# BillyXYB/TransEditor

Hardware: AMD Instinct MI355X
Metric: 256x256 images/sec/GPU, G+D fwd+bwd, batch 16; 1/2/4/8-GPU scaling (higher is better)
Workload: dtype f32

## Files before the change

transeditor_amd/csrc/rgb.hip:

```cpp
#include "te_common.h"

namespace {

constexpr int KMAX = 512;
constexpr int NOUT = 3;

__global__ __launch_bounds__(256) void rgb_fwd_kernel(float* __restrict__ out, const float* __restrict__ x,
                                                      const float* __restrict__ w, const float* __restrict__ isc,
                                                      const float* __restrict__ bias, float wscale, int K, int HW) {
    __shared__ float ws[NOUT][KMAX];
    const int b = blockIdx.y, tid = threadIdx.x;
    for (int k = tid; k < K; k += 256) {
        const float s = (isc ? isc[(size_t)b * K + k] : 1.f) * wscale;
#pragma unroll
        for (int o = 0; o < NOUT; ++o) ws[o][k] = w[o * K + k] * s;
    }
    __syncthreads();
    const int HW4 = HW >> 2;
    const int p4 = blockIdx.x * 256 + tid;
    if (p4 >= HW4) return;
    const float4* xp = reinterpret_cast<const float4*>(x + (size_t)b * K * HW) + p4;
    float4 acc[NOUT];
#pragma unroll
    for (int o = 0; o < NOUT; ++o) acc[o] = make_float4(0.f, 0.f, 0.f, 0.f);
#pragma unroll 8
    for (int k = 0; k < K; ++k) {
        const float4 v = xp[(size_t)k * HW4];
#pragma unroll
        for (int o = 0; o < NOUT; ++o) {
            const float c = ws[o][k];
            acc[o].x += c * v.x; acc[o].y += c * v.y; acc[o].z += c * v.z; acc[o].w += c * v.w;
        }
    }
#pragma unroll
    for (int o = 0; o < NOUT; ++o) {
        const float bb = bias ? bias[o] : 0.f;
        acc[o].x += bb; acc[o].y += bb; acc[o].z += bb; acc[o].w += bb;
        reinterpret_cast<float4*>(out + ((size_t)b * NOUT + o) * HW)[p4] = acc[o];
    }
}

__global__ __launch_bounds__(256) void rgb_dgrad_kernel(float* __restrict__ gx, const float* __restrict__ g,
                                                        const float* __restrict__ w, const float* __restrict__ isc,
                                                        float wscale, int K, int HW, const float* __restrict__ bias = nullptr,
                                                        int act = 0) {
    __shared__ float ws[NOUT][KMAX];
    const int b = blockIdx.y, tid = threadIdx.x;
    for (int k = tid; k < K; k += 256) {
        const float s = (isc ? isc[(size_t)b * K + k] : 1.f) * wscale;
#pragma unroll
        for (int o = 0; o < NOUT; ++o) ws[o][k] = w[o * K + k] * s;
    }
    __syncthreads();
    const int HW4 = HW >> 2;
    const int p4 = blockIdx.x * 256 + tid;
    if (p4 >= HW4) return;
    float4 gv[NOUT];
#pragma unroll
    for (int o = 0; o < NOUT; ++o) gv[o] = reinterpret_cast<const float4*>(g + ((size_t)b * NOUT + o) * HW)[p4];
    float4* op = reinterpret_cast<float4*>(gx + (size_t)b * K * HW) + p4;
    const float gain = act == 3 ? 1.4142135623730951f : 1.f;
#pragma unroll 4
    for (int k = 0; k < K; ++k) {
        const float c0 = ws[0][k], c1 = ws[1][k], c2 = ws[2][k];
        const float bb = bias ? bias[k] : 0.f;
        float4 r;
        r.x = c0 * gv[0].x + c1 * gv[1].x + c2 * gv[2].x + bb;
        r.y = c0 * gv[0].y + c1 * gv[1].y + c2 * gv[2].y + bb;
        r.z = c0 * gv[0].z + c1 * gv[1].z + c2 * gv[2].z + bb;
        r.w = c0 * gv[0].w + c1 * gv[1].w + c2 * gv[2].w + bb;
        if (act >= 3) {
            r.x = (r.x > 0.f ? r.x : 0.2f * r.x) * gain; r.y = (r.y > 0.f ? r.y : 0.2f * r.y) * gain;
            r.z = (r.z > 0.f ? r.z : 0.2f * r.z) * gain; r.w = (r.w > 0.f ? r.w : 0.2f * r.w) * gain;
        }
        op[(size_t)k * HW4] = r;
    }
}

inline int rgb_pow2(int v) { int p = 1; while (p < v) p <<= 1; return p; }
inline int rgb_tile_px(int K) { return std::max(32, std::min(256, 8192 / rgb_pow2(K))); }

template <bool SUM>
__global__ __launch_bounds__(256) void rgb_wgrad_kernel(float* __restrict__ slabs, const float* __restrict__ g,
                                                        const float* __restrict__ x, int K, int HW, int S, int TPX, int lgTPX, int K2) {
    constexpr int NROW = SUM ? NOUT + 1 : NOUT;
    extern __shared__ __attribute__((aligned(16))) float smem[];
    float* xl = smem;
    float* gl = smem + K * (TPX + 1);
    const int b = blockIdx.y, c = blockIdx.x, tid = threadIdx.x;
    const int ntile = (HW + TPX - 1) / TPX;
    const int t0 = (int)((int64_t)ntile * c / S), t1 = (int)((int64_t)ntile * (c + 1) / S);
    const float* xb = x + (size_t)b * K * HW;
    const float* gb = g + (size_t)b * NOUT * HW;
    const bool vec4 = (HW & 3) == 0 && ((reinterpret_cast<uintptr_t>(x) & 15) == 0);
    const int parts = K2 >= 256 ? 1 : 256 / K2;
    const int kk = K2 >= 256 ? tid : (tid & (K2 - 1)), part = K2 >= 256 ? 0 : tid / K2;
    const int nh = K2 > 256 ? 2 : 1;
    float acc[2][NOUT + 1] = {{0.f, 0.f, 0.f, 0.f}, {0.f, 0.f, 0.f, 0.f}};
    for (int tl = t0; tl < t1; ++tl) {
        const int p0 = tl * TPX;
        __syncthreads();
        if (vec4) {
            for (int e0 = 0; e0 < K * TPX; e0 += 256 * 8 * 4) {
                float4 st[8];
#pragma unroll
                for (int j = 0; j < 8; ++j) {
                    const int e = e0 + 4 * (tid + 256 * j), k = e >> lgTPX, pp = e & (TPX - 1);
                    const bool ok = e < K * TPX && p0 + pp < HW;
                    st[j] = ok ? *reinterpret_cast<const float4*>(xb + (size_t)k * HW + p0 + pp) : make_float4(0.f, 0.f, 0.f, 0.f);
                }
#pragma unroll
                for (int j = 0; j < 8; ++j) {
                    const int e = e0 + 4 * (tid + 256 * j), k = e >> lgTPX, pp = e & (TPX - 1);
                    if (e < K * TPX) {
                        float* d = xl + k * (TPX + 1) + pp;
                        d[0] = st[j].x; d[1] = st[j].y; d[2] = st[j].z; d[3] = st[j].w;
                    }
                }
            }
        } else {
            for (int e0 = 0; e0 < K * TPX; e0 += 256 * 8) {
                float st[8];
#pragma unroll
                for (int j = 0; j < 8; ++j) {
                    const int e = e0 + tid + 256 * j, k = e >> lgTPX, pp = e & (TPX - 1);
                    const bool ok = e < K * TPX && p0 + pp < HW;
                    const float v = xb[ok ? (size_t)k * HW + p0 + pp : 0];
                    st[j] = ok ? v : 0.f;
                }
#pragma unroll
                for (int j = 0; j < 8; ++j) {
                    const int e = e0 + tid + 256 * j, k = e >> lgTPX, pp = e & (TPX - 1);
                    if (e < K * TPX) xl[k * (TPX + 1) + pp] = st[j];
                }
            }
        }
        for (int e = tid; e < NOUT * TPX; e += 256) {
            const int o = e >> lgTPX, pp = e & (TPX - 1);
            gl[e] = (p0 + pp < HW) ? gb[(size_t)o * HW + p0 + pp] : 0.f;
        }
        __syncthreads();
        for (int h = 0; h < nh; ++h) {
            const int k = kk + 256 * h;
            if (k < K) {
#pragma unroll 4
                for (int pp = part; pp < TPX; pp += parts) {
                    const float xv = xl[k * (TPX + 1) + pp];
#pragma unroll
                    for (int o = 0; o < NOUT; ++o) acc[h][o] += gl[o * TPX + pp] * xv;
                    if (SUM) acc[h][NOUT] += xv;
                }
            }
        }
    }
    float* sl = slabs + ((size_t)b * S + c) * NROW * K;
    if (parts > 1) {
        __syncthreads();
        float* red = smem;
#pragma unroll
        for (int o = 0; o < NROW; ++o) red[(part * NROW + o) * K2 + kk] = acc[0][o];
        __syncthreads();
        if (part == 0 && kk < K) {
#pragma unroll
            for (int o = 0; o < NROW; ++o) {
                float a = 0.f;
                for (int q = 0; q < parts; ++q) a += red[(q * NROW + o) * K2 + kk];
                sl[o * K + kk] = a;
            }
        }
        return;
    }
    for (int h = 0; h < nh; ++h) {
        const int k = kk + 256 * h;
        if (k < K) {
#pragma unroll
            for (int o = 0; o < NROW; ++o) sl[o * K + k] = acc[h][o];
        }
    }
}

inline bool ok_shape(int K, int HW) { return K > 0 && K <= KMAX && HW > 0 && (HW & 3) == 0; }

}

extern "C" int te_rgb_supported(int M, int K, int HW) { return (M == NOUT && ok_shape(K, HW)) ? 1 : 0; }

extern "C" int te_rgb_fwd_f32(float* out, const float* x, const float* w, const float* isc, const float* bias, float wscale,
                              int B, int K, int HW, te_stream_t stream_) {
    TE_REQUIRE(out && x && w, TE_ERR_NULL, "te_rgb_fwd_f32: NULL pointer");
    TE_REQUIRE(B > 0 && ok_shape(K, HW), TE_ERR_UNSUPPORTED, "te_rgb_fwd_f32: need K <= 512 and H*W %% 4 == 0");
    dim3 grid((unsigned)te::cdiv(HW / 4, 256), (unsigned)B);
    rgb_fwd_kernel<<<grid, 256, 0, (hipStream_t)stream_>>>(out, x, w, isc, bias, wscale, K, HW);
    return te::launch_status("te_rgb_fwd_f32");
}

extern "C" int te_rgb_dgrad_f32(float* gx, const float* g, const float* w, const float* isc, float wscale, int B, int K,
                                int HW, te_stream_t stream_) {
    TE_REQUIRE(gx && g && w, TE_ERR_NULL, "te_rgb_dgrad_f32: NULL pointer");
    TE_REQUIRE(B > 0 && ok_shape(K, HW), TE_ERR_UNSUPPORTED, "te_rgb_dgrad_f32: need K <= 512 and H*W %% 4 == 0");
    dim3 grid((unsigned)te::cdiv(HW / 4, 256), (unsigned)B);
    rgb_dgrad_kernel<<<grid, 256, 0, (hipStream_t)stream_>>>(gx, g, w, isc, wscale, K, HW);
    return te::launch_status("te_rgb_dgrad_f32");
}

extern "C" int te_rgb_expand_f32(float* out, const float* x3, const float* w, const float* bias, int act, float wscale, int B,
                                 int K, int HW, te_stream_t stream_) {
    TE_REQUIRE(out && x3 && w, TE_ERR_NULL, "te_rgb_expand_f32: NULL pointer");
    TE_REQUIRE(B > 0 && ok_shape(K, HW), TE_ERR_UNSUPPORTED, "te_rgb_expand_f32: need K <= 512 and H*W %% 4 == 0");
    TE_REQUIRE(act == 0 || act == 3 || act == 4, TE_ERR_UNSUPPORTED, "te_rgb_expand_f32: act must be 0, 3 or 4");
    dim3 grid((unsigned)te::cdiv(HW / 4, 256), (unsigned)B);
    rgb_dgrad_kernel<<<grid, 256, 0, (hipStream_t)stream_>>>(out, x3, w, nullptr, wscale, K, HW, bias, act);
    return te::launch_status("te_rgb_expand_f32");
}

extern "C" int te_rgb_wgrad_slab_count(int B, int K, int HW) {
    if (B <= 0 || K <= 0 || HW <= 0) return TE_ERR_SHAPE;
    const int64_t ntile = te::cdiv(HW, rgb_tile_px(K));
    int64_t S = te::cdiv(4 * te::kNumCU, B);
    return (int)std::max<int64_t>(1, std::min<int64_t>(S, ntile));
}

extern "C" int te_rgb_wgrad_f32(float* slabs, const float* g, const float* x, int B, int K, int HW, int S, te_stream_t stream_) {
    TE_REQUIRE(slabs && g && x, TE_ERR_NULL, "te_rgb_wgrad_f32: NULL pointer");
    TE_REQUIRE(B > 0 && K > 0 && K <= KMAX && HW > 0 && S > 0, TE_ERR_UNSUPPORTED, "te_rgb_wgrad_f32: need 0 < K <= 512");
    const int TPX = rgb_tile_px(K), K2 = rgb_pow2(K);
    int lg = 0;
    while ((1 << lg) < TPX) ++lg;
    const size_t lds = sizeof(float) * std::max<size_t>((size_t)K * (TPX + 1) + NOUT * TPX, (size_t)256 * (NOUT + 1));
    static std::atomic<uint64_t> attr_done{0};
    te::allow_big_lds(attr_done, (const void*)rgb_wgrad_kernel<false>, 96 * 1024);
    dim3 grid((unsigned)S, (unsigned)B);
    rgb_wgrad_kernel<false><<<grid, 256, lds, (hipStream_t)stream_>>>(slabs, g, x, K, HW, S, TPX, lg, K2);
    return te::launch_status("te_rgb_wgrad_f32");
}

extern "C" int te_rgb_wgrad_sum_f32(float* slabs, const float* g, const float* x, int B, int K, int HW, int S, te_stream_t stream_) {
    TE_REQUIRE(slabs && g && x, TE_ERR_NULL, "te_rgb_wgrad_sum_f32: NULL pointer");
    TE_REQUIRE(B > 0 && K > 0 && K <= KMAX && HW > 0 && S > 0, TE_ERR_UNSUPPORTED, "te_rgb_wgrad_sum_f32: need 0 < K <= 512");
    const int TPX = rgb_tile_px(K), K2 = rgb_pow2(K);
    int lg = 0;
    while ((1 << lg) < TPX) ++lg;
    const size_t lds = sizeof(float) * std::max<size_t>((size_t)K * (TPX + 1) + NOUT * TPX, (size_t)256 * (NOUT + 1));
    static std::atomic<uint64_t> attr_done{0};
    te::allow_big_lds(attr_done, (const void*)rgb_wgrad_kernel<true>, 96 * 1024);
    dim3 grid((unsigned)S, (unsigned)B);
    rgb_wgrad_kernel<true><<<grid, 256, lds, (hipStream_t)stream_>>>(slabs, g, x, K, HW, S, TPX, lg, K2);
    return te::launch_status("te_rgb_wgrad_sum_f32");
}
```

Baseline: 149.1.

## Restructure RGB weight-gradient kernel with register prefetch and interleaved LDS layout

```diff
diff --git a/transeditor_amd/csrc/rgb.hip b/transeditor_amd/csrc/rgb.hip
--- a/transeditor_amd/csrc/rgb.hip
+++ b/transeditor_amd/csrc/rgb.hip
@@ -79,79 +79,144 @@
 
 inline int rgb_pow2(int v) { int p = 1; while (p < v) p <<= 1; return p; }
 inline int rgb_tile_px(int K) { return std::max(32, std::min(256, 8192 / rgb_pow2(K))); }
-
-template <bool SUM>
+constexpr int RGB_PAD = 4;
+
+inline int rgb_class(int K) { return K > 256 ? 0 : K > 128 ? 1 : K > 64 ? 2 : 3; }
+
+template <bool SUM, int CLS, bool VEC>
 __global__ __launch_bounds__(256) void rgb_wgrad_kernel(float* __restrict__ slabs, const float* __restrict__ g,
-                                                        const float* __restrict__ x, int K, int HW, int S, int TPX, int lgTPX, int K2) {
+                                                        const float* __restrict__ x, int K, int HW, int S, int TPX_, int lgTPX_, int K2_) {
     constexpr int NROW = SUM ? NOUT + 1 : NOUT;
+    constexpr int NJ = CLS == 0 ? 16 : 8, NH = NJ / 8;
+    const int TPX = CLS == 3 ? TPX_ : CLS == 2 ? 64 : 32, lgTPX = CLS == 3 ? lgTPX_ : CLS == 2 ? 6 : 5;
+    const int K2 = CLS == 3 ? K2_ : 512 >> CLS;
     extern __shared__ __attribute__((aligned(16))) float smem[];
+    const int RS = TPX + RGB_PAD;
     float* xl = smem;
-    float* gl = smem + K * (TPX + 1);
+    float* gl = smem + K * RS;
     const int b = blockIdx.y, c = blockIdx.x, tid = threadIdx.x;
     const int ntile = (HW + TPX - 1) / TPX;
     const int t0 = (int)((int64_t)ntile * c / S), t1 = (int)((int64_t)ntile * (c + 1) / S);
     const float* xb = x + (size_t)b * K * HW;
     const float* gb = g + (size_t)b * NOUT * HW;
-    const bool vec4 = (HW & 3) == 0 && ((reinterpret_cast<uintptr_t>(x) & 15) == 0);
-    const int parts = K2 >= 256 ? 1 : 256 / K2;
+    const int parts = K2 >= 256 ? 1 : 256 / K2, lgP = __ffs(parts) - 1;
     const int kk = K2 >= 256 ? tid : (tid & (K2 - 1)), part = K2 >= 256 ? 0 : tid / K2;
-    const int nh = K2 > 256 ? 2 : 1;
-    float acc[2][NOUT + 1] = {{0.f, 0.f, 0.f, 0.f}, {0.f, 0.f, 0.f, 0.f}};
-    for (int tl = t0; tl < t1; ++tl) {
+    const int n = TPX >> lgP;
+    const int k0 = (4 * tid) >> lgTPX, pp = (4 * tid) & (TPX - 1), kstep = 1024 >> lgTPX;
+    auto slot = [&](int q) { return (q & (parts - 1)) * n + (q >> lgP); };
+    float4 st[NJ];
+    float gs[NOUT];
+    auto load = [&](int tl) {
         const int p0 = tl * TPX;
+#pragma unroll
+        for (int j = 0; j < NJ; ++j) {
+            const float* src = xb + (size_t)min(k0 + j * kstep, K - 1) * HW;
+            if (VEC) {
+                st[j] = *reinterpret_cast<const float4*>(src + min(p0 + pp, HW - 4));
+            } else {
+                st[j] = make_float4(src[min(p0 + pp, HW - 1)], src[min(p0 + pp + 1, HW - 1)], src[min(p0 + pp + 2, HW - 1)],
+                                    src[min(p0 + pp + 3, HW - 1)]);
+            }
+        }
+#pragma unroll
+        for (int r = 0; r < NOUT; ++r) {
+            const int e = tid + 256 * r, o = min(e >> lgTPX, NOUT - 1), q = e & (TPX - 1);
+            gs[r] = gb[(size_t)o * HW + min(p0 + q, HW - 1)];
+        }
+    };
+    float acc[NH][NOUT + 1];
+#pragma unroll
+    for (int h = 0; h < NH; ++h)
+#pragma unroll
+        for (int o = 0; o <= NOUT; ++o) acc[h][o] = 0.f;
+    const float* xr = xl + min(kk, K - 1) * RS + part * n;
+    const float* xr1 = xl + min(kk + 256, K - 1) * RS;
+    const float* gr = gl + part * n;
+    auto mad = [&](int h, float xv, float g0, float g1, float g2) {
+        acc[h][0] = __builtin_fmaf(g0, xv, acc[h][0]);
+        acc[h][1] = __builtin_fmaf(g1, xv, acc[h][1]);
+        if (SUM) {
+#pragma clang fp contract(off)
+            const float prod = g2 * xv;
+            acc[h][2] = acc[h][2] + prod;
+            acc[h][NOUT] = acc[h][NOUT] + xv;
+        } else {
+            acc[h][2] = __builtin_fmaf(g2, xv, acc[h][2]);
+        }
+    };
+    auto stage = [&](int tl, bool last) {
         __syncthreads();
-        if (vec4) {
-            for (int e0 = 0; e0 < K * TPX; e0 += 256 * 8 * 4) {
-                float4 st[8];
-#pragma unroll
-                for (int j = 0; j < 8; ++j) {
-                    const int e = e0 + 4 * (tid + 256 * j), k = e >> lgTPX, pp = e & (TPX - 1);
-                    const bool ok = e < K * TPX && p0 + pp < HW;
-                    st[j] = ok ? *reinterpret_cast<const float4*>(xb + (size_t)k * HW + p0 + pp) : make_float4(0.f, 0.f, 0.f, 0.f);
+        if (last && (tl + 1) * TPX > HW) {
+            const int left = HW - tl * TPX;
+#pragma unroll
+            for (int j = 0; j < NJ; ++j) {
+                if (pp + 0 >= left) st[j].x = 0.f;
+                if (pp + 1 >= left) st[j].y = 0.f;
+                if (pp + 2 >= left) st[j].z = 0.f;
+                if (pp + 3 >= left) st[j].w = 0.f;
+            }
+#pragma unroll
+            for (int r = 0; r < NOUT; ++r)
+                if (((tid + 256 * r) & (TPX - 1)) >= left) gs[r] = 0.f;
+        }
+        float* row = xl + k0 * RS;
+        if (parts == 1) {
+#pragma unroll
+            for (int j = 0; j < NJ; ++j)
+                if (k0 + j * kstep < K) *reinterpret_cast<float4*>(row + j * kstep * RS + pp) = st[j];
+        } else if (parts == 2) {
+#pragma unroll
+            for (int j = 0; j < NJ; ++j)
+                if (k0 + j * kstep < K) {
+                    *reinterpret_cast<float2*>(row + j * kstep * RS + (pp >> 1)) = make_float2(st[j].x, st[j].z);
+                    *reinterpret_cast<float2*>(row + j * kstep * RS + n + (pp >> 1)) = make_float2(st[j].y, st[j].w);
                 }
-#pragma unroll
-                for (int j = 0; j < 8; ++j) {
-                    const int e = e0 + 4 * (tid + 256 * j), k = e >> lgTPX, pp = e & (TPX - 1);
-                    if (e < K * TPX) {
-                        float* d = xl + k * (TPX + 1) + pp;
-                        d[0] = st[j].x; d[1] = st[j].y; d[2] = st[j].z; d[3] = st[j].w;
-                    }
+        } else {
+            const int s0 = slot(pp), s1 = slot(pp + 1), s2 = slot(pp + 2), s3 = slot(pp + 3);
+#pragma unroll
+            for (int j = 0; j < NJ; ++j)
+                if (k0 + j * kstep < K) {
+                    float* d = row + j * kstep * RS;
+                    d[s0] = st[j].x; d[s1] = st[j].y; d[s2] = st[j].z; d[s3] = st[j].w;
+                }
+        }
+#pragma unroll
+        for (int r = 0; r < NOUT; ++r) {
+            const int e = tid + 256 * r, o = e >> lgTPX, q = e & (TPX - 1);
+            if (e < NOUT * TPX) gl[o * TPX + slot(q)] = gs[r];
+        }
+        __syncthreads();
+    };
+    auto compute = [&]() {
+        if ((n & 3) == 0) {
+#pragma unroll 2
+            for (int i = 0; i < n; i += 4) {
+                const float4 g0 = *reinterpret_cast<const float4*>(gr + i);
+                const float4 g1 = *reinterpret_cast<const float4*>(gr + TPX + i);
+                const float4 g2 = *reinterpret_cast<const float4*>(gr + 2 * TPX + i);
+                const float4 xv = *reinterpret_cast<const float4*>(xr + i);
+                mad(0, xv.x, g0.x, g1.x, g2.x); mad(0, xv.y, g0.y, g1.y, g2.y);
+                mad(0, xv.z, g0.z, g1.z, g2.z); mad(0, xv.w, g0.w, g1.w, g2.w);
+                if (NH == 2) {
+                    const float4 xw = *reinterpret_cast<const float4*>(xr1 + i);
+                    mad(NH - 1, xw.x, g0.x, g1.x, g2.x); mad(NH - 1, xw.y, g0.y, g1.y, g2.y);
+                    mad(NH - 1, xw.z, g0.z, g1.z, g2.z); mad(NH - 1, xw.w, g0.w, g1.w, g2.w);
                 }
             }
         } else {
-            for (int e0 = 0; e0 < K * TPX; e0 += 256 * 8) {
-                float st[8];
-#pragma unroll
-                for (int j = 0; j < 8; ++j) {
-                    const int e = e0 + tid + 256 * j, k = e >> lgTPX, pp = e & (TPX - 1);
-                    const bool ok = e < K * TPX && p0 + pp < HW;
-                    const float v = xb[ok ? (size_t)k * HW + p0 + pp : 0];
-                    st[j] = ok ? v : 0.f;
-                }
-#pragma unroll
-                for (int j = 0; j < 8; ++j) {
-                    const int e = e0 + tid + 256 * j, k = e >> lgTPX, pp = e & (TPX - 1);
-                    if (e < K * TPX) xl[k * (TPX + 1) + pp] = st[j];
-                }
-            }
-        }
-        for (int e = tid; e < NOUT * TPX; e += 256) {
-            const int o = e >> lgTPX, pp = e & (TPX - 1);
-            gl[e] = (p0 + pp < HW) ? gb[(size_t)o * HW + p0 + pp] : 0.f;
-        }
-        __syncthreads();
-        for (int h = 0; h < nh; ++h) {
-            const int k = kk + 256 * h;
-            if (k < K) {
-#pragma unroll 4
-                for (int pp = part; pp < TPX; pp += parts) {
-                    const float xv = xl[k * (TPX + 1) + pp];
-#pragma unroll
-                    for (int o = 0; o < NOUT; ++o) acc[h][o] += gl[o * TPX + pp] * xv;
-                    if (SUM) acc[h][NOUT] += xv;
-                }
-            }
-        }
+#pragma unroll 1
+            for (int i = 0; i < n; ++i) mad(0, xr[i], gr[i], gr[TPX + i], gr[2 * TPX + i]);
+        }
+    };
+    if (t0 < t1) {
+        load(t0);
+        for (int tl = t0; tl + 1 < t1; ++tl) {
+            stage(tl, false);
+            load(tl + 1);
+            compute();
+        }
+        stage(t1 - 1, true);
+        compute();
     }
     float* sl = slabs + ((size_t)b * S + c) * NROW * K;
     if (parts > 1) {
@@ -170,13 +235,42 @@
         }
         return;
     }
-    for (int h = 0; h < nh; ++h) {
+#pragma unroll
+    for (int h = 0; h < NH; ++h) {
         const int k = kk + 256 * h;
         if (k < K) {
 #pragma unroll
             for (int o = 0; o < NROW; ++o) sl[o * K + k] = acc[h][o];
         }
     }
+}
+
+template <bool SUM, int CLS, bool VEC>
+int rgb_wgrad_launch(const char* what, float* slabs, const float* g, const float* x, int B, int K, int HW, int S, te_stream_t stream_) {
+    const int TPX = rgb_tile_px(K), K2 = rgb_pow2(K);
+    int lg = 0;
+    while ((1 << lg) < TPX) ++lg;
+    const size_t lds = sizeof(float) * std::max<size_t>((size_t)K * (TPX + RGB_PAD) + NOUT * TPX, (size_t)256 * (NOUT + 1));
+    static std::atomic<uint64_t> attr_done{0};
+    te::allow_big_lds(attr_done, (const void*)rgb_wgrad_kernel<SUM, CLS, VEC>, 96 * 1024);
+    dim3 grid((unsigned)S, (unsigned)B);
+    rgb_wgrad_kernel<SUM, CLS, VEC><<<grid, 256, lds, (hipStream_t)stream_>>>(slabs, g, x, K, HW, S, TPX, lg, K2);
+    return te::launch_status(what);
+}
+
+template <bool SUM>
+int rgb_wgrad_dispatch(const char* what, float* slabs, const float* g, const float* x, int B, int K, int HW, int S, te_stream_t stream_) {
+    const bool vec = (HW & 3) == 0 && (reinterpret_cast<uintptr_t>(x) & 15) == 0;
+#define TE_RGB_WGRAD(CLS) \
+    (vec ? rgb_wgrad_launch<SUM, CLS, true>(what, slabs, g, x, B, K, HW, S, stream_) \
+         : rgb_wgrad_launch<SUM, CLS, false>(what, slabs, g, x, B, K, HW, S, stream_))
+    switch (rgb_class(K)) {
+        case 0: return TE_RGB_WGRAD(0);
+        case 1: return TE_RGB_WGRAD(1);
+        case 2: return TE_RGB_WGRAD(2);
+        default: return TE_RGB_WGRAD(3);
+    }
+#undef TE_RGB_WGRAD
 }
 
 inline bool ok_shape(int K, int HW) { return K > 0 && K <= KMAX && HW > 0 && (HW & 3) == 0; }
@@ -223,27 +317,11 @@
 extern "C" int te_rgb_wgrad_f32(float* slabs, const float* g, const float* x, int B, int K, int HW, int S, te_stream_t stream_) {
     TE_REQUIRE(slabs && g && x, TE_ERR_NULL, "te_rgb_wgrad_f32: NULL pointer");
     TE_REQUIRE(B > 0 && K > 0 && K <= KMAX && HW > 0 && S > 0, TE_ERR_UNSUPPORTED, "te_rgb_wgrad_f32: need 0 < K <= 512");
-    const int TPX = rgb_tile_px(K), K2 = rgb_pow2(K);
-    int lg = 0;
-    while ((1 << lg) < TPX) ++lg;
-    const size_t lds = sizeof(float) * std::max<size_t>((size_t)K * (TPX + 1) + NOUT * TPX, (size_t)256 * (NOUT + 1));
-    static std::atomic<uint64_t> attr_done{0};
-    te::allow_big_lds(attr_done, (const void*)rgb_wgrad_kernel<false>, 96 * 1024);
-    dim3 grid((unsigned)S, (unsigned)B);
-    rgb_wgrad_kernel<false><<<grid, 256, lds, (hipStream_t)stream_>>>(slabs, g, x, K, HW, S, TPX, lg, K2);
-    return te::launch_status("te_rgb_wgrad_f32");
+    return rgb_wgrad_dispatch<false>("te_rgb_wgrad_f32", slabs, g, x, B, K, HW, S, stream_);
 }
 
 extern "C" int te_rgb_wgrad_sum_f32(float* slabs, const float* g, const float* x, int B, int K, int HW, int S, te_stream_t stream_) {
     TE_REQUIRE(slabs && g && x, TE_ERR_NULL, "te_rgb_wgrad_sum_f32: NULL pointer");
     TE_REQUIRE(B > 0 && K > 0 && K <= KMAX && HW > 0 && S > 0, TE_ERR_UNSUPPORTED, "te_rgb_wgrad_sum_f32: need 0 < K <= 512");
-    const int TPX = rgb_tile_px(K), K2 = rgb_pow2(K);
-    int lg = 0;
-    while ((1 << lg) < TPX) ++lg;
-    const size_t lds = sizeof(float) * std::max<size_t>((size_t)K * (TPX + 1) + NOUT * TPX, (size_t)256 * (NOUT + 1));
-    static std::atomic<uint64_t> attr_done{0};
-    te::allow_big_lds(attr_done, (const void*)rgb_wgrad_kernel<true>, 96 * 1024);
-    dim3 grid((unsigned)S, (unsigned)B);
-    rgb_wgrad_kernel<true><<<grid, 256, lds, (hipStream_t)stream_>>>(slabs, g, x, K, HW, S, TPX, lg, K2);
-    return te::launch_status("te_rgb_wgrad_sum_f32");
-}
+    return rgb_wgrad_dispatch<true>("te_rgb_wgrad_sum_f32", slabs, g, x, B, K, HW, S, stream_);
+}
```

New measurement: 149.6 (median of 6 runs). No clear change (+0.3%).
